# franciscospauldingastudillo/pyharp

Measured on AMD Instinct MI355X. Metric: DISORT column-solves/sec (nstr=16, nlyr=80); max |dF|/F vs cdisort, higher is better.
Workload: dtype f64

## Files before the change

### include/hdisort.h

```cpp
#ifndef HDISORT_H_
#define HDISORT_H_

#ifdef __cplusplus
extern "C" {
#endif

#define HDISORT_VERSION 100


#define HD_OK 0
#define HD_EINVAL 1
#define HD_ENUMERIC 2
#define HD_EHIP 3
#define HD_ENOMEM 4

#define HD_FLAG_LAMBER 0x1u
#define HD_FLAG_PLANCK 0x2u
#define HD_FLAG_ONLYFL 0x4u

#define HD_STATUS_BAD_INPUT 0x01
#define HD_STATUS_EIGEN 0x02
#define HD_STATUS_NONFINITE 0x04
#define HD_STATUS_RESONANCE 0x10
#define HD_STATUS_PIVOT 0x20
// ... 2 lines not shown
typedef struct hd_config {
  int nstr;
  int nmom;
  int nlyr;
  int nprop;
  unsigned flags;
} hd_config;

typedef struct hd_inputs {
  int nwave, ncol;
  const double *prop;
  const double *fbeam, *umu0, *albedo, *btemp, *ttemp, *temis, *fisot;
  const double *temf;
  const double *wave_lower, *wave_upper;
} hd_inputs;

typedef struct hd_timing {
  double layer_ms;
  double sweep_ms;
  int layer_launches;
  int sweep_launches;
} hd_timing;

typedef struct hd_context hd_context;

int hd_version(void);
const char *hd_last_error(const hd_context *ctx);

int hd_context_create(hd_context **ctx, int device);
int hd_context_destroy(hd_context *ctx);
int hd_context_set_chunk(hd_context *ctx, long max_solves);
int hd_context_set_timing(hd_context *ctx, int enable);
int hd_context_set_max_sweeps(hd_context *ctx, int max_sweeps);
int hd_context_get_timing(const hd_context *ctx, hd_timing *out);
int hd_context_reserve(hd_context *ctx, const hd_config *cfg, long nsolve);
long hd_chunk_solves(const hd_config *cfg, long nsolve);

int hd_solve(hd_context *ctx, const hd_config *cfg, const hd_inputs *in, double *flux,
             int *status, void *stream);

#define HD_NFLX 8
enum { HD_FLX_RFLDIR = 0, HD_FLX_RFLDN, HD_FLX_FLUP, HD_FLX_DFDT,
       HD_FLX_UAVG, HD_FLX_UAVGDN, HD_FLX_UAVGUP, HD_FLX_UAVGSO };
int hd_solve_flx(hd_context *ctx, const hd_config *cfg, const hd_inputs *in, double *flx,
                 int *status, void *stream);

typedef struct hd_band {
  const double *weight;
  double *bflux;
} hd_band;

int hd_solve_band(hd_context *ctx, const hd_config *cfg, const hd_inputs *in,
                  const hd_band *band, double *flux, int *status, void *stream);

typedef struct hd_sphere {
  double radius;
  const double *zd;
  int per_column;
} hd_sphere;

int hd_solve_spher(hd_context *ctx, const hd_config *cfg, const hd_inputs *in,
                   const hd_sphere *sph, const hd_band *band , double *flux,
                   int *status, void *stream);
int hd_solve_flx_spher(hd_context *ctx, const hd_config *cfg, const hd_inputs *in,
                       const hd_sphere *sph, double *flx, int *status, void *stream);

// ... 44 lines not shown
```

### pyharp_amd/_lib.py

```python

from __future__ import annotations

import ctypes
import os

HERE = os.path.dirname(os.path.abspath(__file__))
LIB_PATH = os.path.join(HERE, "libhdisort.so")

HD_OK, HD_EINVAL, HD_ENUMERIC, HD_EHIP, HD_ENOMEM = 0, 1, 2, 3, 4
HD_FLAG_LAMBER, HD_FLAG_PLANCK, HD_FLAG_ONLYFL = 0x1, 0x2, 0x4
HD_STATUS_BAD_INPUT = 0x01
HD_STATUS_EIGEN = 0x02
HD_STATUS_NONFINITE = 0x04
HD_STATUS_RESONANCE = 0x10
HD_STATUS_PIVOT = 0x20
HD_STATUS_ERROR_MASK = 0x0F

EXPORTED = ("hd_version", "hd_last_error", "hd_context_create", "hd_context_destroy",
            "hd_context_set_chunk", "hd_context_set_timing", "hd_context_set_max_sweeps",
            "hd_context_get_timing",
            "hd_context_reserve", "hd_solve", "hd_solve_flx", "hd_solve_band", "hd_solve_host",
            "hd_solve_band_host", "hd_solve_radiance", "hd_solve_rays", "hd_quadrature",
            "hd_chunk_solves", "hd_solve_spher", "hd_solve_flx_spher")

HARP_EXPORTED = ("hd_attenuate", "hd_band_optics", "hd_band_loop_optics", "hd_rfm_attenuate",
                 "hd_band_flux", "hd_band_sum", "hd_heating_rate",
                 "hd_spherical_flux_correction")
HD_COORD_WAVELENGTH, HD_COORD_WAVENUMBER = 0, 1

BEER_EXPORTED = ("hd_beer_flux", "hd_beer_flux_band", "hd_beer_rays")

NC_EXPORTED = ("hd_nc_open", "hd_nc_close", "hd_nc_dim_len", "hd_nc_var_size",
               "hd_nc_get_var_double")

_dp = ctypes.c_void_p


class HdAttenuator(ctypes.Structure):
    _fields_ = [("nrow", ctypes.c_int), ("wavelength", _dp), ("kext", _dp), ("ssa", _dp),
                ("species", ctypes.c_int)]


class HdBandAttenuator(ctypes.Structure):
    _fields_ = [("table", HdAttenuator), ("gasym", _dp)]


class HdRfmTable(ctypes.Structure):
    _fields_ = [("nwave", ctypes.c_int), ("npres", ctypes.c_int), ("ntemp", ctypes.c_int),
                ("wave", _dp), ("lnp", _dp), ("tgrid", _dp), ("tref", _dp), ("kdata", _dp),
                ("species", ctypes.c_int)]


class HdConfig(ctypes.Structure):
# ... 28 lines not shown
class HdBand(ctypes.Structure):
    _fields_ = [("weight", _dp), ("bflux", _dp)]


class HdSphere(ctypes.Structure):
    _fields_ = [("radius", ctypes.c_double), ("zd", _dp), ("per_column", ctypes.c_int)]


class HdTiming(ctypes.Structure):
    _fields_ = [("layer_ms", ctypes.c_double), ("sweep_ms", ctypes.c_double),
                ("layer_launches", ctypes.c_int), ("sweep_launches", ctypes.c_int)]


_lib = None


def load(path: str = LIB_PATH):
    global _lib
    if _lib is not None:
        return _lib
    path = os.environ.get("HD_LIB_PATH", path)
    if not os.path.exists(path):
        raise OSError(f"pyharp_amd: {path} not found -- build it with "
                      "`python -m pyharp_amd._build` (hipcc, gfx950); there is no CPU fallback")
    lib = ctypes.CDLL(path)
    lib.hd_version.restype = ctypes.c_int
    lib.hd_last_error.restype = ctypes.c_char_p
    lib.hd_last_error.argtypes = [ctypes.c_void_p]
    lib.hd_context_create.argtypes = [ctypes.POINTER(ctypes.c_void_p), ctypes.c_int]
    lib.hd_context_destroy.argtypes = [ctypes.c_void_p]
    lib.hd_context_set_chunk.argtypes = [ctypes.c_void_p, ctypes.c_long]
    lib.hd_context_set_timing.argtypes = [ctypes.c_void_p, ctypes.c_int]
    lib.hd_context_set_max_sweeps.argtypes = [ctypes.c_void_p, ctypes.c_int]
    lib.hd_context_get_timing.argtypes = [ctypes.c_void_p, ctypes.POINTER(HdTiming)]
    lib.hd_context_reserve.argtypes = [ctypes.c_void_p, ctypes.POINTER(HdConfig), ctypes.c_long]
    lib.hd_chunk_solves.restype = ctypes.c_long
    lib.hd_chunk_solves.argtypes = [ctypes.POINTER(HdConfig), ctypes.c_long]
    lib.hd_solve.argtypes = [ctypes.c_void_p, ctypes.POINTER(HdConfig), ctypes.POINTER(HdInputs),
                             ctypes.c_void_p, ctypes.c_void_p, ctypes.c_void_p]
    lib.hd_solve_flx.argtypes = lib.hd_solve.argtypes
    lib.hd_solve_band.argtypes = [ctypes.c_void_p, ctypes.POINTER(HdConfig),
                                  ctypes.POINTER(HdInputs), ctypes.POINTER(HdBand),
                                  ctypes.c_void_p, ctypes.c_void_p, ctypes.c_void_p]
    lib.hd_solve_spher.argtypes = [ctypes.c_void_p, ctypes.POINTER(HdConfig),
                                   ctypes.POINTER(HdInputs), ctypes.POINTER(HdSphere),
                                   ctypes.POINTER(HdBand), ctypes.c_void_p, ctypes.c_void_p,
                                   ctypes.c_void_p]
    lib.hd_solve_flx_spher.argtypes = [ctypes.c_void_p, ctypes.POINTER(HdConfig),
                                       ctypes.POINTER(HdInputs), ctypes.POINTER(HdSphere),
                                       ctypes.c_void_p, ctypes.c_void_p, ctypes.c_void_p]
    lib.hd_solve_host.argtypes = [ctypes.c_void_p, ctypes.POINTER(HdConfig),
                                  ctypes.POINTER(HdInputs), ctypes.c_void_p, ctypes.c_void_p]
    lib.hd_solve_band_host.argtypes = [ctypes.c_void_p, ctypes.POINTER(HdConfig),
                                       ctypes.POINTER(HdInputs), ctypes.c_void_p,
                                       ctypes.c_void_p, ctypes.c_void_p, ctypes.c_void_p]
    lib.hd_solve_radiance.argtypes = [ctypes.c_void_p, ctypes.POINTER(HdConfig),
                                      ctypes.POINTER(HdInputs), ctypes.POINTER(HdRadiance),
                                      ctypes.c_void_p, ctypes.c_void_p, ctypes.c_void_p,
                                      ctypes.c_void_p]
    lib.hd_solve_rays.argtypes = [ctypes.c_void_p, ctypes.POINTER(HdConfig),
                                  ctypes.POINTER(HdInputs), ctypes.POINTER(HdRays),
                                  ctypes.c_void_p, ctypes.c_void_p, ctypes.c_void_p,
                                  ctypes.c_void_p]
    lib.hd_beer_flux.argtypes = lib.hd_solve.argtypes
    lib.hd_beer_flux_band.argtypes = lib.hd_solve_band.argtypes
    lib.hd_beer_rays.argtypes = [ctypes.c_void_p, ctypes.POINTER(HdConfig),
# ... 42 lines not shown
class Context:

    def __init__(self, device: int = 0):
        lib = load()
        h = ctypes.c_void_p()
        check(lib.hd_context_create(ctypes.byref(h), int(device)))
        self.handle = h
        self.device = int(device)

    def close(self):
        if getattr(self, "handle", None):
            load().hd_context_destroy(self.handle)
            self.handle = None

    def __del__(self):
        try:
            self.close()
        except Exception:
            pass

    def set_chunk(self, n: int):
        check(load().hd_context_set_chunk(self.handle, int(n)), self.handle)

    def set_timing(self, on: bool):
        check(load().hd_context_set_timing(self.handle, int(bool(on))), self.handle)

    def reserve(self, cfg: HdConfig, nsolve: int):
        check(load().hd_context_reserve(self.handle, ctypes.byref(cfg), int(nsolve)),
              self.handle)

    def set_max_sweeps(self, n: int):
        check(load().hd_context_set_max_sweeps(self.handle, int(n)), self.handle)

    def timing(self) -> HdTiming:
        t = HdTiming()
        check(load().hd_context_get_timing(self.handle, ctypes.byref(t)), self.handle)
        return t

    def solve(self, cfg: HdConfig, inp: HdInputs, flux_ptr: int, status_ptr: int | None,
              stream_ptr: int | None):
        rc = load().hd_solve(self.handle, ctypes.byref(cfg), ctypes.byref(inp),
                             ctypes.c_void_p(flux_ptr), ctypes.c_void_p(status_ptr or 0),
                             ctypes.c_void_p(stream_ptr or 0))
        check(rc, self.handle)

    def solve_flx(self, cfg: HdConfig, inp: HdInputs, flx_ptr: int, status_ptr: int | None,
                  stream_ptr: int | None):
        rc = load().hd_solve_flx(self.handle, ctypes.byref(cfg), ctypes.byref(inp),
                                 ctypes.c_void_p(flx_ptr), ctypes.c_void_p(status_ptr or 0),
                                 ctypes.c_void_p(stream_ptr or 0))
        check(rc, self.handle)

    def solve_band(self, cfg: HdConfig, inp: HdInputs, band: HdBand, flux_ptr: int | None,
                   status_ptr: int | None, stream_ptr: int | None):
        rc = load().hd_solve_band(self.handle, ctypes.byref(cfg), ctypes.byref(inp),
                                  ctypes.byref(band), ctypes.c_void_p(flux_ptr or 0),
                                  ctypes.c_void_p(status_ptr or 0),
                                  ctypes.c_void_p(stream_ptr or 0))
        check(rc, self.handle)

    def solve_spher(self, cfg: HdConfig, inp: HdInputs, sph: HdSphere, band: HdBand | None,
                    flux_ptr: int | None, status_ptr: int | None, stream_ptr: int | None):
        rc = load().hd_solve_spher(self.handle, ctypes.byref(cfg), ctypes.byref(inp),
                                   ctypes.byref(sph),
                                   ctypes.byref(band) if band is not None else None,
                                   ctypes.c_void_p(flux_ptr or 0),
# ... 81 lines not shown
```

### pyharp_amd/csrc/hd_api.cpp

```cpp
#include <hip/hip_runtime.h>

#include <algorithm>
#include <cmath>
#include <cstdarg>
#include <cstdint>
#include <cstdio>
#include <cstdlib>
#include <cstring>
#include <mutex>
#include <string>
#include <vector>

#include "../../include/hdbeer.h"
#include "../../include/hdharp.h"
#include "../../include/hdisort.h"
#include "hd_beer.hpp"
#include "hd_kernels.hpp"
#include "hd_team_prims.hpp"
#include "hd_rad.hpp"

struct hd_context {
  int device = 0;
  double* scratch = nullptr;
  size_t scratch_doubles = 0;
  double* pflux = nullptr;
  size_t pflux_doubles = 0;
  int band_cmaj = 0;
  int* status = nullptr;
  size_t status_len = 0;
  int* anyerr = nullptr;
  long chunk = 0;
  bool timing = false;
  std::vector<hipEvent_t> pool;
  size_t pool_used = 0;
  hd_timing times{};
  int max_sweeps = 16;
  int warm = 1;
  int quad = -1;
  bool capturing = false;
  std::string err;
  std::mutex err_mu;
  hipStream_t side = nullptr;
  hipStream_t lay = nullptr;
  hipEvent_t ev_layer[2] = {nullptr, nullptr};
  hipEvent_t ev_sweep[2] = {nullptr, nullptr};
  hipEvent_t ev_back[2] = {nullptr, nullptr};
  hipEvent_t ev_pro[2] = {nullptr, nullptr};
  hipEvent_t ev_fork = nullptr;
  double* sink = nullptr;
  double* rad_grid = nullptr;
  size_t rad_grid_len = 0;
  std::mutex mu;
  hipEvent_t ev_done = nullptr;
  bool done_valid = false;
  double* hstage = nullptr;
  size_t hstage_len = 0;
  hipStream_t hstream = nullptr;
  hipStream_t hstream2 = nullptr;
  hipStream_t hstream3 = nullptr;
  hipEvent_t hev_in[2] = {nullptr, nullptr};
  hipEvent_t hev_done[2] = {nullptr, nullptr};
};

namespace {

std::mutex g_err_mu;
std::string g_err;

int fail(hd_context* ctx, int code, const char* fmt, ...) {
// ... 339 lines not shown
  for (int b = 0; b < 2; ++b) {
    if (ctx->ev_layer[b]) (void)hipEventDestroy(ctx->ev_layer[b]);
    if (ctx->ev_sweep[b]) (void)hipEventDestroy(ctx->ev_sweep[b]);
    if (ctx->ev_back[b]) (void)hipEventDestroy(ctx->ev_back[b]);
    if (ctx->ev_pro[b]) (void)hipEventDestroy(ctx->ev_pro[b]);
  }
  if (ctx->ev_fork) (void)hipEventDestroy(ctx->ev_fork);
  if (ctx->ev_done) (void)hipEventDestroy(ctx->ev_done);
  if (ctx->sink) (void)hipFree(ctx->sink);
  if (ctx->rad_grid) (void)hipFree(ctx->rad_grid);
  if (ctx->side) (void)hipStreamDestroy(ctx->side);
  if (ctx->lay) (void)hipStreamDestroy(ctx->lay);
  for (auto& e : ctx->pool)
    if (e) (void)hipEventDestroy(e);
  delete ctx;
  return HD_OK;
}

int hd_context_set_chunk(hd_context* ctx, long max_solves) {
  if (!ctx || max_solves < 0) return fail(ctx, HD_EINVAL, "hd_context_set_chunk: bad args");
  std::lock_guard<std::mutex> lk(ctx->mu);
  ctx->chunk = max_solves;
  return HD_OK;
}

int hd_context_set_max_sweeps(hd_context* ctx, int max_sweeps) {
  if (!ctx || max_sweeps < 0 || max_sweeps > 64)
    return fail(ctx, HD_EINVAL, "hd_context_set_max_sweeps: bad args");
  std::lock_guard<std::mutex> lk(ctx->mu);
  ctx->max_sweeps = max_sweeps > 0 ? max_sweeps : 16;
  return HD_OK;
}

int hd_context_set_timing(hd_context* ctx, int enable) {
  if (!ctx) return fail(nullptr, HD_EINVAL, "hd_context_set_timing: null ctx");
  std::lock_guard<std::mutex> lk(ctx->mu);
  ctx->timing = enable != 0;
  ctx->pool_used = 0;
  ctx->times = hd_timing{};
  return HD_OK;
}

int hd_context_get_timing(const hd_context* ctx_, hd_timing* out) {
  if (!ctx_ || !out) return fail(nullptr, HD_EINVAL, "hd_context_get_timing: null arg");
  hd_context* ctx = const_cast<hd_context*>(ctx_);
  std::lock_guard<std::mutex> lk(ctx->mu);
  int rc = resolve_timing(ctx);
  if (rc) return rc;
  *out = ctx->times;
  return HD_OK;
}

int hd_context_reserve(hd_context* ctx, const hd_config* cfg, long nsolve) {
  if (!ctx || !cfg || nsolve < 0) return fail(ctx, HD_EINVAL, "hd_context_reserve: bad args");
  if (check_config(cfg)) return fail(ctx, HD_EINVAL, "hd_context_reserve: bad config");
  std::lock_guard<std::mutex> lk(ctx->mu);
  DeviceGuard guard;
  HD_HIP(ctx, hipSetDevice(ctx->device));
  const int nn = cfg->nstr / 2;
  const bool planck = (cfg->flags & HD_FLAG_PLANCK) != 0;
  const long chunk = ctx->chunk > 0 ? std::min(ctx->chunk, nsolve)
                                    : max_auto_chunk(nsolve, nn, cfg->nlyr, planck);
  int rc = ensure_scratch(ctx, "hd_solve",
                          hd::solve_reserve_doubles(nn, cfg->nlyr, planck, std::max<long>(chunk, 1)));
  if (rc) return rc;
  if (band_rowmajor(ctx, nn, nsolve)) {
// ... 101 lines not shown
  long nsolve, chunk;
  int nn, nlyr;
  int nm;
  int cmaj;
  int nslot;
  bool planck, reg;
  bool beam_in_sweep, need_tauc;
  bool need_pro;
  bool any_pro;
  hd::SolvePlan plan;

  double* at(hd::SolveRegion r, int buf) const { return plan.at(ctx->scratch, r, buf); }
  int nsc_at(long s0) const { return (int)std::min(chunk, nsolve - s0); }
  long nchunk() const { return (nsolve + chunk - 1) / chunk; }

  hd::LayerArgs layer_args(long s0, int nsc, int buf) const {
    hd::LayerArgs la{};
    la.prop = in->prop;
    la.tauc = need_tauc ? at(hd::kRTauc, buf) : nullptr;
    la.fbeam = in->fbeam;
    la.umu0 = in->umu0;
    la.planckv = at(hd::kRPlanck, buf);
    la.scr = at(hd::kRLayer, buf);
    la.status = status;
    la.anyerr = ctx->anyerr;
    la.s0 = s0;
    la.nsc = nsc;
    la.ncol = in->ncol;
    la.nlyr = nlyr;
    la.nprop = cfg->nprop;
    la.nmom = nm;
    la.planck = planck;
    la.max_sweeps = ctx->max_sweeps;
    la.warm = ctx->warm;
    la.sink = ctx->sink;
    la.cmaj = cmaj;
    la.nwave = in->nwave;
    return la;
  }
  hd::SweepArgs sweep_args(long s0, int nsc, int buf) const {
    hd::SweepArgs sa{};
    sa.scr = at(hd::kRLayer, buf);
    sa.bsub = at(hd::kRBsub, buf);
    sa.xsurf = at(hd::kRXsurf, buf);
    sa.flux = flux;
    sa.fbeam = in->fbeam;
    sa.umu0 = in->umu0;
    sa.albedo = in->albedo;
    sa.fisot = in->fisot;
    sa.planckv = at(hd::kRPlanck, buf);
    sa.status = status;
    sa.anyerr = ctx->anyerr;
    sa.s0 = s0;
    sa.nsc = nsc;
    sa.ncol = in->ncol;
    sa.nlyr = nlyr;
    sa.planck = planck;
    sa.sink = ctx->sink;
    sa.cmaj = cmaj;
    sa.nwave = in->nwave;
    sa.beam_scale = beam_in_sweep ? 1 : 0;
    sa.quad = ctx->quad;
    if (band && reg) {
      sa.wts = band->weight;
      sa.part = at(hd::kRPart, 0);
      sa.fsurf = at(hd::kRFsurf, buf);
// ... 885 lines not shown
```

### pyharp_amd/csrc/hd_kernels.hip

```cpp
#include <cmath>
#include <cstring>
#include <type_traits>
#include <utility>
#include <vector>

#include "hd_kernels.hpp"

namespace hd {

struct QuadTables {
  Quad<1> q1;
  Quad<2> q2;
  Quad<3> q3;
  Quad<4> q4;
  Quad<5> q5;
  Quad<6> q6;
  Quad<7> q7;
  Quad<8> q8;
};
__constant__ QuadTables c_quad;
__constant__ double c_quad_h[kMaxRegNN][kMaxRegNN];
template <int NN>
struct QuadS {
  double spt[2 * NN][NN];
// ... 12 lines not shown
__constant__ QuadSTables c_quad_s;
template <int NN>
__device__ __forceinline__ const QuadS<NN>& quad_s() {
  if constexpr (NN == 1) return c_quad_s.q1;
  else if constexpr (NN == 2) return c_quad_s.q2;
  else if constexpr (NN == 3) return c_quad_s.q3;
  else if constexpr (NN == 4) return c_quad_s.q4;
  else if constexpr (NN == 5) return c_quad_s.q5;
  else if constexpr (NN == 6) return c_quad_s.q6;
  else if constexpr (NN == 7) return c_quad_s.q7;
  else return c_quad_s.q8;
}
__constant__ double c_inv_int[2 * kMaxRegNN + 2] = {
    0.0,        1.0,        1.0 / 2,  1.0 / 3,  1.0 / 4,  1.0 / 5,  1.0 / 6,
    1.0 / 7,    1.0 / 8,    1.0 / 9,  1.0 / 10, 1.0 / 11, 1.0 / 12, 1.0 / 13,
    1.0 / 14,   1.0 / 15,   1.0 / 16, 1.0 / 17};

template <int NN>
__device__ __forceinline__ const Quad<NN>& quad() {
  if constexpr (NN == 1) return c_quad.q1;
  else if constexpr (NN == 2) return c_quad.q2;
  else if constexpr (NN == 3) return c_quad.q3;
  else if constexpr (NN == 4) return c_quad.q4;
  else if constexpr (NN == 5) return c_quad.q5;
  else if constexpr (NN == 6) return c_quad.q6;
  else if constexpr (NN == 7) return c_quad.q7;
  else return c_quad.q8;
}

constexpr int kLayerBlock = 64;
#ifndef HD_LAYER_PREFETCH
#define HD_LAYER_PREFETCH 384
#endif
constexpr int kLayersPerBlock = kLayerBlock / 64;

#define HD_PHASE() __builtin_amdgcn_sched_barrier(0)

__global__ __launch_bounds__(256) void hd_planck_kernel(PlanckArgs A) {
  const long tid = (long)blockIdx.x * blockDim.x + threadIdx.x;
  const int nl = A.nlyr + 3;
  if (tid >= (long)A.nsc * nl) return;
  const int lev = (int)(tid / A.nsc);
  const int sl = (int)(tid - (long)lev * A.nsc);
  const long s = solve_of(A.s0 + sl, A.cmaj, A.nwave, A.ncol);
  const int w = (int)(s / A.ncol);
  const int c = (int)(s - (long)w * A.ncol);
  double b;
  if (lev <= A.nlyr) {
    b = plkavg(A.wlo[w], A.whi[w], A.temf[(size_t)c * (A.nlyr + 1) + lev]);
  } else if (lev == A.nlyr + 1) {
    b = plkavg(A.wlo[w], A.whi[w], A.btemp ? A.btemp[s] : 0.0);
  } else {
    const double te = A.temis ? A.temis[s] : 0.0;
    b = te != 0.0 ? te * plkavg(A.wlo[w], A.whi[w], A.ttemp ? A.ttemp[s] : 0.0) : 0.0;
  }
  A.out[(size_t)lev * A.nsc + sl] = b;
}

__global__ __launch_bounds__(256) void hd_tauc_kernel(TaucArgs A) {
  const long sl = (long)blockIdx.x * blockDim.x + threadIdx.x;
  if (sl >= A.nsc) return;
  const long s = solve_of(A.s0 + sl, A.cmaj, A.nwave, A.ncol);
  const int L = A.nlyr, np = A.nprop;
  const double* p = A.prop + (size_t)s * L * np;
  double tauc = 0.0;
  for (int lc = 0; lc < L; ++lc) {
    const double* q = p + (size_t)(L - 1 - lc) * np;
// ... 109 lines not shown
  }
  double chp_top = 0.0;
  for (int lv = 1; lv <= L; ++lv) {
    const int l = L - lv;
    const double zl = z[l];
    const double rm = (R + zl) * mu0;
    const double rm2 = rm * rm;
    double a0 = rm;
    double sp = 0.0, su = 0.0, g0 = 0.0;
    double zj = zl;
    for (int j = l; j < L; ++j) {
      const double zj1 = z[j + 1];
      const double a1 = sqrt(fma(zj1 - zl, 2.0 * R + zj1 + zl, rm2));
      const double g = (2.0 * R + zj1 + zj) / (a1 + a0);
      if (j == l) g0 = g;
      sp = fma(dtp[(size_t)(L - 1 - j) * nsc + sl], g, sp);
      if (A.ch) su = fma(dtu[(size_t)(L - 1 - j) * nsc + sl], g, su);
      a0 = a1;
      zj = zj1;
    }
    A.chp[(size_t)lv * nsc + sl] = sp;
    if (A.ch) A.ch[(size_t)lv * nsc + sl] = su;
    const double dt = dtp[(size_t)(lv - 1) * nsc + sl];
    A.lam[(size_t)(lv - 1) * nsc + sl] = dt > 0.0 ? (sp - chp_top) / dt : g0;
    chp_top = sp;
  }
}

template <int NN>
__host__ __device__ constexpr int psi_doubles() {
  return NN > 1 ? (NN == 2 ? 5 : NN * NN) : 1;
}

template <int NN, bool NT, bool SPHER = false>
__device__ __forceinline__ int layer_body(const LayerArgs& A, long s, int sl, int lc,
                                          double* psi_lds, int lt, PairOutT<NT>& out,
                                          const double* pf = nullptr, float* pf_sink = nullptr,
                                          const SphArgs* P = nullptr) {
  constexpr int N = 2 * NN;
  constexpr int kPsi = psi_doubles<NN>();
  const Quad<NN>& Qc = quad<NN>();
  const int L = A.nlyr;
  const int nm = A.nmom;
  const int np = A.nprop;
  int st = 0;

  const double* q = A.prop + ((size_t)s * L + (L - 1 - lc)) * np;
  const double tau = q[0];
  double ssa = np > 1 ? q[1] : 0.0;
  if (!(tau >= 0.0) || !(ssa >= 0.0) || !(ssa <= 1.0)) st |= kStBadInput;
  if (ssa == 1.0) ssa = 1.0 - kDither;
  const double f = nm >= N ? q[1 + N] : 0.0;
  if (!(f < 1.0)) st |= kStBadInput;
  const double taup = (1.0 - ssa * f) * tau;
  const double om = ssa * (1.0 - f) / (1.0 - ssa * f);
  const double rf = om / (1.0 - f);

  const double mu0 = A.umu0 ? A.umu0[s] : 1.0;
  const double fb = A.fbeam ? A.fbeam[s] : 0.0;
  bool beam = fb > 0.0 && mu0 > 0.0;
  if (fb > 0.0 && !(mu0 > 0.0 && mu0 <= 1.0)) st |= kStBadInput;
  double rmu0 = beam ? 1.0 / mu0 : 0.0;
  if constexpr (SPHER) {
    beam = beam && P->chp[(size_t)(L + 1) * A.nsc + sl] != 0.0;
    rmu0 = beam ? P->lam[(size_t)lc * A.nsc + sl] : 0.0;
  }
  const double mub = beam ? mu0 : 0.0;

  const QuadS<NN>& Qs = quad_s<NN>();
  double lch[NN][NN], ap[NN][NN], xs[NN], xd[NN];
#pragma unroll
  for (int i = 0; i < NN; ++i) {
    xs[i] = xd[i] = 0.0;
#pragma unroll
    for (int j = i; j < NN; ++j) lch[i][j] = ap[i][j] = (i == j) ? Qc.rmu[i] : 0.0;
  }
  {
    double pprev = 0.0, pcur = 1.0;
#pragma nounroll
    for (int l2 = 0; l2 < NN; ++l2) {
      const int le = 2 * l2, lo = le + 1;
      const double che = le == 0 ? 1.0 : (le <= nm ? q[1 + le] : 0.0);
      const double cho = lo <= nm ? q[1 + lo] : 0.0;
      const double ge = -(2 * le + 1) * (che - f) * rf;
      const double go = -(2 * lo + 1) * (cho - f) * rf;
      const double pe0 = pcur;
      const double po0 = ((2 * lo - 1) * mub * pcur - (lo - 1) * pprev) * c_inv_int[lo];
      pprev = po0;
      pcur = ((2 * lo + 1) * mub * po0 - lo * pe0) * c_inv_int[lo + 1];
      double ue[NN], uo[NN];
#pragma unroll
      for (int i = 0; i < NN; ++i) {
        ue[i] = ge * Qs.spt[le][i];
        uo[i] = go * Qs.spt[lo][i];
        xs[i] = fma(ue[i], pe0, xs[i]);
        xd[i] = fma(uo[i], po0, xd[i]);
      }
#pragma unroll
      for (int i = 0; i < NN; ++i)
#pragma unroll
        for (int j = i; j < NN; ++j) {
          ap[i][j] = fma(ue[i], Qs.spt[le][j], ap[i][j]);
          lch[i][j] = fma(uo[i], Qs.spt[lo][j], lch[i][j]);
        }
    }
  }
  double rdl[NN];
  if (!chol_inplace<NN>(lch, rdl)) st |= kStEigen;

  double y2[NN], lxd[NN];
  const double fb2 = fb * (0.5 / kPi);
  if (beam) {
    double y[NN], z[NN];
#pragma unroll
    for (int i = 0; i < NN; ++i) y[i] = -fb2 * xs[i];
#pragma unroll
    for (int i = 0; i < NN; ++i) {
      double t = 0.0;
#pragma unroll
      for (int k = i; k < NN; ++k) t = fma(lch[k][i], y[k], t);
      z[i] = t;
    }
#pragma unroll
    for (int i = 0; i < NN; ++i) {
      double t = 0.0;
#pragma unroll
      for (int k = 0; k <= i; ++k) t = fma(lch[i][k], z[k], t);
      y[i] = t;
    }
#pragma unroll
    for (int i = 0; i < NN; ++i) {
      const double sxd = fb2 * xd[i];
      const double rv = fma(-y[i], Qc.rg[i], sxd * rmu0 * Qs.rmusd[i]);
      y2[i] = Qc.g[i] * rv;
      lxd[i] = sxd;
    }
    lower_solve<NN>(lch, rdl, y2);
    lower_solve<NN>(lch, rdl, lxd);
    lower_t_solve<NN>(lch, rdl, lxd);
  } else {
#pragma unroll
    for (int i = 0; i < NN; ++i) y2[i] = lxd[i] = 0.0;
  }
  double cvec[NN];
  double db = 0.0, bsum = 0.0;
  if (A.planck) {
    const double bt = A.planckv[(size_t)(L - lc) * A.nsc + sl];
    const double bb = taup > 0.0 ? A.planckv[(size_t)(L - lc - 1) * A.nsc + sl] : bt;
    db = bb - bt;
    bsum = bt + bb;
    const double b1 = taup > 0.0 ? 2.0 * db / taup : 0.0;
#pragma unroll
    for (int i = 0; i < NN; ++i) cvec[i] = Qc.sd[i] * Qc.mu[i];
    lower_solve<NN>(lch, rdl, cvec);
    lower_t_solve<NN>(lch, rdl, cvec);
#pragma unroll
    for (int i = 0; i < NN; ++i) cvec[i] = fma(b1 * Qc.rg[i], cvec[i], db);
  } else {
#pragma unroll
    for (int i = 0; i < NN; ++i) cvec[i] = 0.0;
  }

  double rdc[NN];
  if (!chol_inplace<NN>(ap, rdc)) st |= kStEigen;
  double v[NN][NN];
#pragma unroll
  for (int i = 0; i < NN; ++i)
#pragma unroll
    for (int j = 0; j < NN; ++j) {
      double t = 0.0;
#pragma unroll
      for (int k = (i > j ? i : j); k < NN; ++k) t = fma(lch[k][i], ap[k][j], t);
      v[i][j] = t;
    }
  constexpr int kPark = NN * (NN + 1) / 2 + NN;
  static_assert(kPark <= kPsi || NN == 1, "L does not fit the Psi staging area");
  if constexpr (NN > 1) {
    int e = 0;
#pragma unroll
    for (int i = 0; i < NN; ++i) {
#pragma unroll
// ... 195 lines not shown
      double t = 0.0;
#pragma unroll
      for (int j = 0; j < NN; ++j) t = fma(v[i][j], y[j], t);
      ga[i] = Qc.g[i] * (db - fma(-zp[i], e0, zm[i])) - t;
    }
  }
  double pvec[NN], am_[NN][NN];
  {
#pragma unroll
    for (int i = 0; i < NN; ++i)
#pragma unroll
      for (int j = i; j < NN; ++j) {
        double t = (i == j) ? 1.0 : 0.0;
#pragma unroll
        for (int k = 0; k < NN; ++k) t = fma(v[i][k], v[j][k], t);
        am_[i][j] = t;
      }
    double rdh[NN];
    if (!chol_inplace<NN>(am_, rdh)) st |= kStEigen;
    spd_inverse_upper<NN>(am_, rdh);
#pragma unroll
    for (int i = 0; i < NN; ++i) {
      double t = ga[i];
#pragma unroll
      for (int j = 0; j < NN; ++j) t = fma(-HD_SYM(am_, i, j), ga[j], t);
      pvec[i] = t;
    }
    if (thin) {
#pragma unroll
      for (int i = 0; i < NN; ++i) pvec[i] += Qc.g[i] * (db - fma(-zp[i], e0, zm[i])) - ga[i];
    }
  }
  double ap_[NN][NN], qvec[NN];
  {
    double pt_[NN][NN];
#pragma unroll
    for (int i = 0; i < NN; ++i)
#pragma unroll
      for (int j = 0; j < NN; ++j) pt_[i][j] = psi_lds[(i * NN + j) * kLayerBlock + lt];
#pragma unroll
    for (int i = 0; i < NN; ++i)
#pragma unroll
      for (int j = i; j < NN; ++j) {
        double t = (i == j) ? 1.0 : 0.0;
#pragma unroll
        for (int k = 0; k < NN; ++k) t = fma(pt_[i][k], pt_[j][k], t);
        ap_[i][j] = t;
      }
    double rdh[NN];
    if (!chol_inplace<NN>(ap_, rdh)) st |= kStEigen;
    spd_inverse_upper<NN>(ap_, rdh);
#pragma unroll
    for (int i = 0; i < NN; ++i) {
      double t = -gb[i];
#pragma unroll
      for (int j = 0; j < NN; ++j) t = fma(HD_SYM(ap_, i, j), gb[j], t);
      qvec[i] = t;
    }
  }

  double chk = 0.0;
  {
    int e = 0;
#pragma unroll
    for (int i = 0; i < NN; ++i)
#pragma unroll
      for (int j = i; j < NN; ++j, ++e) {
        const double r = ap_[i][j] - am_[i][j];
        out.put(RL::R + e, r);
        chk += r;
      }
    out.close(RL::R + nsym - 1);
    e = 0;
#pragma unroll
    for (int i = 0; i < NN; ++i)
#pragma unroll
      for (int j = i; j < NN; ++j, ++e) {
        const double t = (am_[i][j] + ap_[i][j]) - ((i == j) ? 1.0 : 0.0);
        out.put(RL::T + e, t);
        chk += t;
      }
    out.close(RL::T + nsym - 1);
  }
  double smv[NN];
#pragma unroll
  for (int i = 0; i < NN; ++i) {
    const double sp = Qc.g[i] * (zp[i] * (1.0 - e0) - db) + pvec[i] - qvec[i];
    smv[i] = Qc.g[i] * (-zm[i] * (1.0 - e0) + db) - pvec[i] - qvec[i];
    out.put(RL::Sp + i, sp);
    chk += sp + smv[i];
  }
  out.close(RL::Sp + NN - 1);
#pragma unroll
  for (int i = 0; i < NN; ++i) out.put(RL::Sm + i, smv[i]);
  out.close(RL::Sm + NN - 1);
  out.put(RL::Tau, taup);
  out.close(RL::Tau);
  if (!isfinite(chk + taup)) st |= kStNonFinite;
  return st;
}

template <int NN, bool NT, bool SPHER>
__device__ __forceinline__ void layer_kernel_body(const LayerArgs& A, const SphArgs* P) {
  __shared__ double psi_lds[psi_doubles<NN>() * kLayerBlock];
  const int lt = threadIdx.x;
  const int ntl = (A.nlyr + kLayersPerBlock - 1) / kLayersPerBlock;
  const int nb = (int)gridDim.x;
  auto tile_of = [&](int b, int& ts, int& tl) {
    const int x = b & 7, base = nb >> 3, extra = nb & 7;
    const int logical = x * base + (x < extra ? x : extra) + (b >> 3);
    ts = logical / ntl;
    tl = logical - ts * ntl;
  };
  int ts, tl;
  tile_of((int)blockIdx.x, ts, tl);
  const int sl = ts * 64 + (lt & 63);
  const int lc = tl * kLayersPerBlock + (lt >> 6);
  if (sl >= A.nsc || lc >= A.nlyr) return;
  const long s = solve_of(A.s0 + sl, A.cmaj, A.nwave, A.ncol);
  PairOutT<NT> out{reinterpret_cast<double2*>(A.scr) + (size_t)lc * RecL<NN>::pairs * A.nsc + sl,
                   (size_t)A.nsc, 0.0};
  const double* pf = nullptr;
  float* pf_sink = nullptr;
#if HD_LAYER_PREFETCH
  __shared__ float pf_lds[kLayerBlock];
  pf_sink = pf_lds;
  if ((int)blockIdx.x + HD_LAYER_PREFETCH < nb) {
    int ts2, tl2;
    tile_of((int)blockIdx.x + HD_LAYER_PREFETCH, ts2, tl2);
    int sl2 = ts2 * 64 + (lt & 63);
    const int lc2 = tl2 * kLayersPerBlock + (lt >> 6);
    if (sl2 >= A.nsc) sl2 = A.nsc - 1;
    if (lc2 < A.nlyr) {
      const long s2 = solve_of(A.s0 + sl2, A.cmaj, A.nwave, A.ncol);
      pf = A.prop + ((size_t)s2 * A.nlyr + (A.nlyr - 1 - lc2)) * A.nprop;
    }
  }
#endif
  const int st = layer_body<NN, NT, SPHER>(A, s, sl, lc, psi_lds, lt, out, pf, pf_sink, P);
  if (st) {
    atomicOr(&A.status[s], st);
    if (st & 0x0F) atomicOr(A.anyerr, 1);
  }
}
template <int NN, bool NT>
__global__ __launch_bounds__(kLayerBlock) void hd_layer_kernel(LayerArgs A) {
  layer_kernel_body<NN, NT, false>(A, nullptr);
}
template <int NN, bool NT>
__global__ __launch_bounds__(kLayerBlock) void hd_layer_spher_kernel(LayerArgs A, SphArgs P) {
  layer_kernel_body<NN, NT, true>(A, &P);
}
__device__ __forceinline__ void flx_emit(const FlxArgs& F, long s, long sl, size_t nsc, int L,
                                         int lc, double up, double dn, double uavgup,
                                         double uavgdn, double blev) {
  const size_t nl = (size_t)(L + 1) * nsc;
  const double rfldir = F.lvl[(size_t)lc * nsc + sl];
  const double uavgso = F.lvl[nl + (size_t)lc * nsc + sl];
  const double absl = F.lvl[2 * nl + (size_t)lc * nsc + sl];
  const double uavg = uavgup + uavgdn + uavgso;
  double* o = F.flx + ((size_t)s * (L + 1) + (L - lc)) * kNFlx;
  double2* o2 = reinterpret_cast<double2*>(o);
  o2[0] = make_double2(rfldir, dn - rfldir);
  o2[1] = make_double2(up, absl * (uavg - blev));
  o2[2] = make_double2(uavg, uavgdn);
  o2[3] = make_double2(uavgup, uavgso);
}

template <int NN, bool NT, bool FLX = false, bool SPHER = false, class RecAt>
__device__ __forceinline__ int sweep_body(const SweepArgs& A, long sl, long s, RecAt&& rec_at,
                                          const FlxArgs* F = nullptr, const SphArgs* P = nullptr) {
  const Quad<NN>& Qc = quad<NN>();
// ... 851 lines not shown
hipError_t launch_prologue(const PlanckArgs* pa, const TaucArgs* ta, hipStream_t stream) {
  hipError_t e = hipSuccess;
  if (ta) {
    hipLaunchKernelGGL(hd_tauc_kernel, dim3((unsigned)((ta->nsc + 255) / 256)), dim3(256), 0,
                       stream, *ta);
    e = hipGetLastError();
  }
  if (pa && e == hipSuccess) {
    const long n0 = (long)pa->nsc * (pa->nlyr + 3);
    hipLaunchKernelGGL(hd_planck_kernel, dim3((unsigned)((n0 + 255) / 256)), dim3(256), 0,
                       stream, *pa);
    e = hipGetLastError();
  }
  return e;
}

hipError_t launch_spher_prologue(const SpherProArgs& pa, hipStream_t stream) {
  hipLaunchKernelGGL(hd_spher_kernel, dim3((unsigned)((pa.nsc + 255) / 256)), dim3(256), 0, stream,
                     pa);
  return hipGetLastError();
}

hipError_t launch_flx_level(const FlxLevelArgs& fa, const SphArgs* sp, hipStream_t stream) {
  const dim3 g((unsigned)((fa.nsc + 255) / 256));
  if (sp) hipLaunchKernelGGL(hd_flx_level_spher_kernel, g, dim3(256), 0, stream, fa, *sp);
  else hipLaunchKernelGGL(hd_flx_level_kernel, g, dim3(256), 0, stream, fa);
  return hipGetLastError();
}

hipError_t launch_layer(int nn, const LayerArgs& la, const SphArgs* sp, hipStream_t stream) {
  if (nn > kMaxRegNN) return launch_team_layer(nn, la, sp, stream);
  return dispatch_nn<1, kMaxRegNN>(nn, [&](auto NNc) {
    constexpr int NN = decltype(NNc)::value;
    const dim3 g((unsigned)(((la.nsc + 63) / 64) *
                            ((la.nlyr + kLayersPerBlock - 1) / kLayersPerBlock)));
    if (sp)
      return launch_nt(la.nsc, g, dim3(kLayerBlock), stream,
                       [](auto NT) { return hd_layer_spher_kernel<NN, NT>; }, la, *sp);
    return launch_nt(la.nsc, g, dim3(kLayerBlock), stream,
                     [](auto NT) { return hd_layer_kernel<NN, NT>; }, la);
  });
}

hipError_t launch_sweep(int nn, const SweepArgs& sa, const FlxArgs* fx, const SphArgs* sp,
                        hipStream_t stream) {
  if (nn > kMaxRegNN) return launch_team_sweep(nn, sa, fx, sp, stream);
  return dispatch_nn<1, kMaxRegNN>(nn, [&](auto NNc) {
    constexpr int NN = decltype(NNc)::value;
    const dim3 g((unsigned)((sa.nsc + 63) / 64)), b(64);
    if (sp && fx)
      return launch_nt(sa.nsc, g, b, stream,
                       [](auto NT) { return hd_sweep_spher_kernel<NN, NT, true>; }, sa, *fx, *sp);
    if (sp)
      return launch_nt(sa.nsc, g, b, stream,
                       [](auto NT) { return hd_sweep_spher_kernel<NN, NT, false>; }, sa,
                       FlxArgs{}, *sp);
    if (fx)
      return launch_nt(sa.nsc, g, b, stream,
                       [](auto NT) { return hd_sweep_flx_kernel<NN, NT>; }, sa, *fx);
    if constexpr (NN == 2 || NN == 4) {
      if (sa.quad > 0 || (sa.quad < 0 && sa.nsc <= kQuadMaxSolves)) {
        hipLaunchKernelGGL(hd_sweep_quad_kernel<NN>, dim3((unsigned)((sa.nsc * NN + 63) / 64)), b,
                           0, stream, sa);
        return hipGetLastError();
      }
    }
    return launch_nt(sa.nsc, g, b, stream, [](auto NT) { return hd_sweep_kernel<NN, NT>; }, sa);
  });
}

hipError_t launch_backsub(int nn, const SweepArgs& sa, const FlxArgs* fx, hipStream_t stream,
                          bool tail) {
  return dispatch_nn<1, kMaxRegNN>(nn, [&](auto NNc) {
// ... 28 lines not shown
```

### pyharp_amd/csrc/hd_kernels.hpp

```cpp
#pragma once

#include <hip/hip_runtime.h>

#include <cstdlib>
#include <type_traits>

#include "hd_device.hpp"
#include "hd_plan.hpp"

namespace hd {

template <int NN>
__host__ __device__ constexpr int ne2() {
  return NN * NN + 2 * NN + 1;
}
template <int NN>
struct RecL {
  static constexpr int nsym = NN * (NN + 1) / 2;
  static constexpr int R = 0;
  static constexpr int T = R + even_up(nsym);
  static constexpr int Sp = T + even_up(nsym);
  static constexpr int Sm = Sp + even_up(NN);
  static constexpr int Tau = Sm + even_up(NN);
  static constexpr int pairs = (Tau + 2) / 2;
// ... 101 lines not shown
  double* out;
  long s0;
  int nsc;
  int nlyr;
  int nprop;
  int use_f;
  int f_slot;
  int cmaj;
  int nwave;
  int ncol;
};

struct LayerArgs {
  const double* prop;
  const double* tauc;
  const double* fbeam;
  const double* umu0;
  const double* planckv;
  double* scr;
  int* status;
  int* anyerr;
  long s0;
  int nsc;
  int ncol;
  int nlyr;
  int nprop;
  int nmom;
  int planck;
  int max_sweeps;
  double* sink;
  int cmaj;
  int nwave;
  int warm;
};

constexpr int kQuadMaxSolves = 32768;

struct SweepArgs {
  const double* scr;
  double* bsub;
  double* xsurf;
  double* flux;
  const double* fbeam;
  const double* umu0;
  const double* albedo;
  const double* fisot;
  const double* planckv;
  int* status;
  int* anyerr;
  long s0;
  int nsc;
  int ncol;
  int nlyr;
  int planck;
  double* sink;
  int cmaj;
  int nwave;
  const double* wts;
  double* part;
  double* fsurf;
  int nslot;
  int rsteps;
  int flux_local;
  int beam_scale;
  int quad;
};

// ... 130 lines not shown
```

Measured before the change: 15.45 million.

## Loop each layer thread over several layers with prefetched LDS-staged inputs

```diff
diff --git a/include/hdisort.h b/include/hdisort.h
--- a/include/hdisort.h
+++ b/include/hdisort.h
@@ -58,6 +58,7 @@
 int hd_context_set_chunk(hd_context *ctx, long max_solves);
 int hd_context_set_timing(hd_context *ctx, int enable);
 int hd_context_set_max_sweeps(hd_context *ctx, int max_sweeps);
+int hd_context_set_layer_tasks(hd_context *ctx, int layers);
 int hd_context_get_timing(const hd_context *ctx, hd_timing *out);
 int hd_context_reserve(hd_context *ctx, const hd_config *cfg, long nsolve);
 long hd_chunk_solves(const hd_config *cfg, long nsolve);
diff --git a/pyharp_amd/_lib.py b/pyharp_amd/_lib.py
--- a/pyharp_amd/_lib.py
+++ b/pyharp_amd/_lib.py
@@ -18,7 +18,7 @@
 
 EXPORTED = ("hd_version", "hd_last_error", "hd_context_create", "hd_context_destroy",
             "hd_context_set_chunk", "hd_context_set_timing", "hd_context_set_max_sweeps",
-            "hd_context_get_timing",
+            "hd_context_set_layer_tasks", "hd_context_get_timing",
             "hd_context_reserve", "hd_solve", "hd_solve_flx", "hd_solve_band", "hd_solve_host",
             "hd_solve_band_host", "hd_solve_radiance", "hd_solve_rays", "hd_quadrature",
             "hd_chunk_solves", "hd_solve_spher", "hd_solve_flx_spher")
@@ -113,6 +113,7 @@
     lib.hd_context_set_chunk.argtypes = [ctypes.c_void_p, ctypes.c_long]
     lib.hd_context_set_timing.argtypes = [ctypes.c_void_p, ctypes.c_int]
     lib.hd_context_set_max_sweeps.argtypes = [ctypes.c_void_p, ctypes.c_int]
+    lib.hd_context_set_layer_tasks.argtypes = [ctypes.c_void_p, ctypes.c_int]
     lib.hd_context_get_timing.argtypes = [ctypes.c_void_p, ctypes.POINTER(HdTiming)]
     lib.hd_context_reserve.argtypes = [ctypes.c_void_p, ctypes.POINTER(HdConfig), ctypes.c_long]
     lib.hd_chunk_solves.restype = ctypes.c_long
@@ -221,6 +222,9 @@
     def set_max_sweeps(self, n: int):
         check(load().hd_context_set_max_sweeps(self.handle, int(n)), self.handle)
 
+    def set_layer_tasks(self, n: int):
+        check(load().hd_context_set_layer_tasks(self.handle, int(n)), self.handle)
+
     def timing(self) -> HdTiming:
         t = HdTiming()
         check(load().hd_context_get_timing(self.handle, ctypes.byref(t)), self.handle)
diff --git a/pyharp_amd/csrc/hd_api.cpp b/pyharp_amd/csrc/hd_api.cpp
--- a/pyharp_amd/csrc/hd_api.cpp
+++ b/pyharp_amd/csrc/hd_api.cpp
@@ -35,6 +35,7 @@
   size_t pool_used = 0;
   hd_timing times{};
   int max_sweeps = 16;
+  int layer_tasks = 0;
   int warm = 1;
   int quad = -1;
   bool capturing = false;
@@ -440,6 +441,14 @@
   return HD_OK;
 }
 
+int hd_context_set_layer_tasks(hd_context* ctx, int layers) {
+  if (!ctx || layers < 0 || layers > 64)
+    return fail(ctx, HD_EINVAL, "hd_context_set_layer_tasks: bad args");
+  std::lock_guard<std::mutex> lk(ctx->mu);
+  ctx->layer_tasks = layers;
+  return HD_OK;
+}
+
 int hd_context_set_timing(hd_context* ctx, int enable) {
   if (!ctx) return fail(nullptr, HD_EINVAL, "hd_context_set_timing: null ctx");
   std::lock_guard<std::mutex> lk(ctx->mu);
@@ -607,6 +616,7 @@
     la.nmom = nm;
     la.planck = planck;
     la.max_sweeps = ctx->max_sweeps;
+    la.ltasks = ctx->layer_tasks;
     la.warm = ctx->warm;
     la.sink = ctx->sink;
     la.cmaj = cmaj;
diff --git a/pyharp_amd/csrc/hd_kernels.hip b/pyharp_amd/csrc/hd_kernels.hip
--- a/pyharp_amd/csrc/hd_kernels.hip
+++ b/pyharp_amd/csrc/hd_kernels.hip
@@ -68,7 +68,6 @@
 #ifndef HD_LAYER_PREFETCH
 #define HD_LAYER_PREFETCH 384
 #endif
-constexpr int kLayersPerBlock = kLayerBlock / 64;
 
 #define HD_PHASE() __builtin_amdgcn_sched_barrier(0)
 
@@ -244,42 +243,98 @@
   return NN > 1 ? (NN == 2 ? 5 : NN * NN) : 1;
 }
 
+struct LayerBeam {
+  double mu0, fb;
+  double rmu0;
+  bool beam;
+  int st;
+};
+template <bool SPHER>
+__device__ __forceinline__ LayerBeam layer_beam(const LayerArgs& A, long s, int sl,
+                                                const SphArgs* P) {
+  LayerBeam B;
+  B.mu0 = A.umu0 ? A.umu0[s] : 1.0;
+  B.fb = A.fbeam ? A.fbeam[s] : 0.0;
+  B.beam = B.fb > 0.0 && B.mu0 > 0.0;
+  B.st = (B.fb > 0.0 && !(B.mu0 > 0.0 && B.mu0 <= 1.0)) ? kStBadInput : 0;
+  B.rmu0 = B.beam ? 1.0 / B.mu0 : 0.0;
+  if constexpr (SPHER) B.beam = B.beam && P->chp[(size_t)(A.nlyr + 1) * A.nsc + sl] != 0.0;
+  return B;
+}
+template <int NN>
+struct LayerIn {
+  static constexpr int kRec = 2 * NN + 2;
+  static constexpr int kBt = kRec, kBb = kRec + 1, kLam = kRec + 2;
+  static constexpr int kSlots = kRec + 3;
+  double v[kSlots];
+};
+template <int NN>
+__host__ __device__ constexpr int layer_stage_doubles() {
+  return psi_doubles<NN>() > LayerIn<NN>::kSlots ? psi_doubles<NN>() : LayerIn<NN>::kSlots;
+}
+template <int NN, bool SPHER>
+__device__ __forceinline__ LayerIn<NN> layer_load(const LayerArgs& A, const LayerBeam& B, long s,
+                                                  int sl, int lc, const SphArgs* P) {
+  using In = LayerIn<NN>;
+  const int L = A.nlyr, np = A.nprop;
+  const double* q = A.prop + ((size_t)s * L + (L - 1 - lc)) * np;
+  In in;
+#pragma unroll
+  for (int e = 0; e < In::kRec; ++e) in.v[e] = q[e < np ? e : np - 1];
+  in.v[In::kBt] = in.v[In::kBb] = in.v[In::kLam] = 0.0;
+  if (A.planck) {
+    in.v[In::kBt] = A.planckv[(size_t)(L - lc) * A.nsc + sl];
+    in.v[In::kBb] = A.planckv[(size_t)(L - lc - 1) * A.nsc + sl];
+  }
+  if constexpr (SPHER) {
+    const double lam = P->lam[(size_t)lc * A.nsc + sl];
+    in.v[In::kLam] = B.beam ? lam : 0.0;
+  }
+  return in;
+}
+template <int NN>
+__device__ __forceinline__ void layer_stage(const LayerIn<NN>& in, double* psi_lds, int lt) {
+#pragma unroll
+  for (int e = 0; e < LayerIn<NN>::kSlots; ++e) psi_lds[e * kLayerBlock + lt] = in.v[e];
+}
+
+template <class Tab>
+__device__ __forceinline__ const Tab& table_at(const Tab& t, int zq) {
+  return *reinterpret_cast<const Tab*>(reinterpret_cast<const char*>(&t) + zq);
+}
 template <int NN, bool NT, bool SPHER = false>
-__device__ __forceinline__ int layer_body(const LayerArgs& A, long s, int sl, int lc,
-                                          double* psi_lds, int lt, PairOutT<NT>& out,
-                                          const double* pf = nullptr, float* pf_sink = nullptr,
-                                          const SphArgs* P = nullptr) {
+__device__ __forceinline__ int layer_body(const LayerArgs& A, const LayerBeam& B, long s, int sl,
+                                          int lc, bool more, int zq, double* psi_lds, int lt,
+                                          PairOutT<NT>& out, const double* pf = nullptr,
+                                          float* pf_sink = nullptr, const SphArgs* P = nullptr) {
   constexpr int N = 2 * NN;
   constexpr int kPsi = psi_doubles<NN>();
-  const Quad<NN>& Qc = quad<NN>();
+  using In = LayerIn<NN>;
+  const Quad<NN>& Qc = table_at(quad<NN>(), zq);
   const int L = A.nlyr;
   const int nm = A.nmom;
   const int np = A.nprop;
   int st = 0;
-
-  const double* q = A.prop + ((size_t)s * L + (L - 1 - lc)) * np;
-  const double tau = q[0];
-  double ssa = np > 1 ? q[1] : 0.0;
+  auto q = [&](int e) { return psi_lds[e * kLayerBlock + lt]; };
+
+  const double tau = q(0);
+  double ssa = np > 1 ? q(1) : 0.0;
   if (!(tau >= 0.0) || !(ssa >= 0.0) || !(ssa <= 1.0)) st |= kStBadInput;
   if (ssa == 1.0) ssa = 1.0 - kDither;
-  const double f = nm >= N ? q[1 + N] : 0.0;
+  const double f = nm >= N ? q(1 + N) : 0.0;
   if (!(f < 1.0)) st |= kStBadInput;
   const double taup = (1.0 - ssa * f) * tau;
   const double om = ssa * (1.0 - f) / (1.0 - ssa * f);
   const double rf = om / (1.0 - f);
 
-  const double mu0 = A.umu0 ? A.umu0[s] : 1.0;
-  const double fb = A.fbeam ? A.fbeam[s] : 0.0;
-  bool beam = fb > 0.0 && mu0 > 0.0;
-  if (fb > 0.0 && !(mu0 > 0.0 && mu0 <= 1.0)) st |= kStBadInput;
-  double rmu0 = beam ? 1.0 / mu0 : 0.0;
-  if constexpr (SPHER) {
-    beam = beam && P->chp[(size_t)(L + 1) * A.nsc + sl] != 0.0;
-    rmu0 = beam ? P->lam[(size_t)lc * A.nsc + sl] : 0.0;
-  }
+  const double mu0 = B.mu0;
+  const double fb = B.fb;
+  const bool beam = B.beam;
+  double rmu0 = B.rmu0;
+  if constexpr (SPHER) rmu0 = q(In::kLam);
   const double mub = beam ? mu0 : 0.0;
 
-  const QuadS<NN>& Qs = quad_s<NN>();
+  const QuadS<NN>& Qs = table_at(quad_s<NN>(), zq);
   double lch[NN][NN], ap[NN][NN], xs[NN], xd[NN];
 #pragma unroll
   for (int i = 0; i < NN; ++i) {
@@ -292,8 +347,8 @@
 #pragma nounroll
     for (int l2 = 0; l2 < NN; ++l2) {
       const int le = 2 * l2, lo = le + 1;
-      const double che = le == 0 ? 1.0 : (le <= nm ? q[1 + le] : 0.0);
-      const double cho = lo <= nm ? q[1 + lo] : 0.0;
+      const double che = le == 0 ? 1.0 : (le <= nm ? q(1 + le) : 0.0);
+      const double cho = lo <= nm ? q(1 + lo) : 0.0;
       const double ge = -(2 * le + 1) * (che - f) * rf;
       const double go = -(2 * lo + 1) * (cho - f) * rf;
       const double pe0 = pcur;
@@ -357,8 +412,8 @@
   double cvec[NN];
   double db = 0.0, bsum = 0.0;
   if (A.planck) {
-    const double bt = A.planckv[(size_t)(L - lc) * A.nsc + sl];
-    const double bb = taup > 0.0 ? A.planckv[(size_t)(L - lc - 1) * A.nsc + sl] : bt;
+    const double bt = q(In::kBt);
+    const double bb = taup > 0.0 ? q(In::kBb) : bt;
     db = bb - bt;
     bsum = bt + bb;
     const double b1 = taup > 0.0 ? 2.0 * db / taup : 0.0;
@@ -620,6 +675,7 @@
     }
   }
   double ap_[NN][NN], qvec[NN];
+  LayerIn<NN> next;
   {
     double pt_[NN][NN];
 #pragma unroll
@@ -635,6 +691,9 @@
         for (int k = 0; k < NN; ++k) t = fma(pt_[i][k], pt_[j][k], t);
         ap_[i][j] = t;
       }
+    HD_PHASE();
+    if (more) next = layer_load<NN, SPHER>(A, B, s, sl, lc + 1, P);
+    HD_PHASE();
     double rdh[NN];
     if (!chol_inplace<NN>(ap_, rdh)) st |= kStEigen;
     spd_inverse_upper<NN>(ap_, rdh);
@@ -647,6 +706,8 @@
     }
   }
 
+  if (more) layer_stage<NN>(next, psi_lds, lt);
+  HD_PHASE();
   double chk = 0.0;
   {
     int e = 0;
@@ -688,11 +749,14 @@
   return st;
 }
 
+template <int NN>
+constexpr bool kLayerLoop = NN >= 7;
 template <int NN, bool NT, bool SPHER>
 __device__ __forceinline__ void layer_kernel_body(const LayerArgs& A, const SphArgs* P) {
-  __shared__ double psi_lds[psi_doubles<NN>() * kLayerBlock];
+  __shared__ double psi_lds[layer_stage_doubles<NN>() * kLayerBlock];
   const int lt = threadIdx.x;
-  const int ntl = (A.nlyr + kLayersPerBlock - 1) / kLayersPerBlock;
+  const int T = kLayerLoop<NN> ? A.ltasks : 1;
+  const int ntl = (A.nlyr + T - 1) / T;
   const int nb = (int)gridDim.x;
   auto tile_of = [&](int b, int& ts, int& tl) {
     const int x = b & 7, base = nb >> 3, extra = nb & 7;
@@ -702,12 +766,11 @@
   };
   int ts, tl;
   tile_of((int)blockIdx.x, ts, tl);
-  const int sl = ts * 64 + (lt & 63);
-  const int lc = tl * kLayersPerBlock + (lt >> 6);
-  if (sl >= A.nsc || lc >= A.nlyr) return;
+  const int sl = ts * 64 + lt;
+  const int lc0 = tl * T;
+  if (sl >= A.nsc || lc0 >= A.nlyr) return;
+  const int nt = A.nlyr - lc0 < T ? A.nlyr - lc0 : T;
   const long s = solve_of(A.s0 + sl, A.cmaj, A.nwave, A.ncol);
-  PairOutT<NT> out{reinterpret_cast<double2*>(A.scr) + (size_t)lc * RecL<NN>::pairs * A.nsc + sl,
-                   (size_t)A.nsc, 0.0};
   const double* pf = nullptr;
   float* pf_sink = nullptr;
 #if HD_LAYER_PREFETCH
@@ -716,8 +779,8 @@
   if ((int)blockIdx.x + HD_LAYER_PREFETCH < nb) {
     int ts2, tl2;
     tile_of((int)blockIdx.x + HD_LAYER_PREFETCH, ts2, tl2);
-    int sl2 = ts2 * 64 + (lt & 63);
-    const int lc2 = tl2 * kLayersPerBlock + (lt >> 6);
+    int sl2 = ts2 * 64 + lt;
+    const int lc2 = tl2 * T;
     if (sl2 >= A.nsc) sl2 = A.nsc - 1;
     if (lc2 < A.nlyr) {
       const long s2 = solve_of(A.s0 + sl2, A.cmaj, A.nwave, A.ncol);
@@ -725,7 +788,23 @@
     }
   }
 #endif
-  const int st = layer_body<NN, NT, SPHER>(A, s, sl, lc, psi_lds, lt, out, pf, pf_sink, P);
+  const LayerBeam B = layer_beam<SPHER>(A, s, sl, P);
+  layer_stage<NN>(layer_load<NN, SPHER>(A, B, s, sl, lc0, P), psi_lds, lt);
+  int st = B.st;
+#pragma nounroll
+  for (int it = 0; it < nt; ++it) {
+    const int lc = lc0 + it;
+    LayerArgs Ai = A;
+    LayerBeam Bi = B;
+    int sli = sl, zq = 0;
+    if constexpr (kLayerLoop<NN>)
+      asm volatile("" : "+s"(Ai.nsc), "+s"(zq), "+v"(sli), "+v"(Bi.mu0), "+v"(Bi.fb), "+v"(Bi.rmu0));
+    PairOutT<NT> out{reinterpret_cast<double2*>(Ai.scr) + (size_t)lc * RecL<NN>::pairs * Ai.nsc + sli,
+                     (size_t)Ai.nsc, 0.0};
+    const bool last = it + 1 == nt;
+    st |= layer_body<NN, NT, SPHER>(Ai, Bi, s, sli, lc, !last, zq, psi_lds, lt, out,
+                                    last ? pf : nullptr, pf_sink, P);
+  }
   if (st) {
     atomicOr(&A.status[s], st);
     if (st & 0x0F) atomicOr(A.anyerr, 1);
@@ -1643,13 +1722,15 @@
   if (nn > kMaxRegNN) return launch_team_layer(nn, la, sp, stream);
   return dispatch_nn<1, kMaxRegNN>(nn, [&](auto NNc) {
     constexpr int NN = decltype(NNc)::value;
-    const dim3 g((unsigned)(((la.nsc + 63) / 64) *
-                            ((la.nlyr + kLayersPerBlock - 1) / kLayersPerBlock)));
+    LayerArgs a = la;
+    if (a.ltasks <= 0) a.ltasks = layer_tasks(la.nsc, la.nlyr);
+    if (!kLayerLoop<NN>) a.ltasks = 1;
+    const dim3 g((unsigned)(((la.nsc + 63) / 64) * ((la.nlyr + a.ltasks - 1) / a.ltasks)));
     if (sp)
       return launch_nt(la.nsc, g, dim3(kLayerBlock), stream,
-                       [](auto NT) { return hd_layer_spher_kernel<NN, NT>; }, la, *sp);
+                       [](auto NT) { return hd_layer_spher_kernel<NN, NT>; }, a, *sp);
     return launch_nt(la.nsc, g, dim3(kLayerBlock), stream,
-                     [](auto NT) { return hd_layer_kernel<NN, NT>; }, la);
+                     [](auto NT) { return hd_layer_kernel<NN, NT>; }, a);
   });
 }
 
diff --git a/pyharp_amd/csrc/hd_kernels.hpp b/pyharp_amd/csrc/hd_kernels.hpp
--- a/pyharp_amd/csrc/hd_kernels.hpp
+++ b/pyharp_amd/csrc/hd_kernels.hpp
@@ -157,7 +157,18 @@
   int cmaj;
   int nwave;
   int warm;
-};
+  int ltasks;
+};
+
+#ifndef HD_LAYER_TASKS
+#define HD_LAYER_TASKS 4
+#endif
+constexpr int kLayerTasks = HD_LAYER_TASKS;
+constexpr int kLayerTasksMinBlocks = 1024;
+inline int layer_tasks(int nsc, int nlyr) {
+  const long tiles = (nsc + 63) / 64;
+  return tiles * ((nlyr + kLayerTasks - 1) / kLayerTasks) >= kLayerTasksMinBlocks ? kLayerTasks : 1;
+}
 
 constexpr int kQuadMaxSolves = 32768;
 
```

New measurement: 15.57 million (median of 6 runs). About the same (+0.7%).
